# Pablete1234/parquet-floor

Measured on AMD Instinct MI355X. Metric: decoded GB/s + rows/s (node), lineitem-shape Snappy+dict, 1/2/4/8 GPUs, higher is better.
Workload: dtype u8; 1 GPU; lineitem SF1 x1 (6001215 rows x 1, 16 cols, 6 row groups of 1Mi rows), Snappy + dictionary, device-resident; row_groups_per_rank=6, compressed_page_bytes_rank0=217870360

## Files before the change

### parquet-floor_amd/csrc/pf_snappy_par.hip

```cpp
#include <hip/hip_runtime.h>


#include "pf_launch.h"
#include "pf_snappy_par.h"

namespace pf {

#ifdef PF_STAMPS
__device__ unsigned long long pf_stamps[16];
#define STAMP_ADD(i, v) atomicAdd(&pf_stamps[i], (unsigned long long)(v))
__device__ unsigned long long pf_cstamps[32];
#define CSTAMP(i, v) atomicAdd(&pf_cstamps[i], (unsigned long long)(v))
extern "C" int pf_debug_cstamps(unsigned long long* out, int n, int reset) {
    if (hipMemcpyFromSymbol(out, HIP_SYMBOL(pf_cstamps), sizeof(unsigned long long) * (n < 32 ? n : 32)) != hipSuccess) return -1;
    if (reset) {
        unsigned long long z[32] = {};
        if (hipMemcpyToSymbol(HIP_SYMBOL(pf_cstamps), z, sizeof z) != hipSuccess) return -1;
    }
    return 0;
}
#define XT_DECL unsigned long long xt_ = __builtin_amdgcn_s_memtime()
#define XT(i) do { const unsigned long long t_ = __builtin_amdgcn_s_memtime(); if (lane == 0) STAMP_ADD(i, t_ - xt_); xt_ = t_; } while (0)
#else
#define STAMP_ADD(i, v) ((void)0)
// ... 985 lines not shown
        for (uint32_t u = 0; u < XST; u++)
            put16(o, a0 + 16 * u, *reinterpret_cast<const u32x4*>(ring + ((a0 + 16 * u) & XRMASK)));
        F += XSLOT;
        nsl += XST;
    }
    return nsl;
}

__device__ __forceinline__ uint32_t dpp_incl_scan(uint32_t v) {
    v += __builtin_amdgcn_update_dpp(0u, v, 0x111, 0xf, 0xf, false);
    v += __builtin_amdgcn_update_dpp(0u, v, 0x112, 0xf, 0xf, false);
    v += __builtin_amdgcn_update_dpp(0u, v, 0x114, 0xf, 0xf, false);
    v += __builtin_amdgcn_update_dpp(0u, v, 0x118, 0xf, 0xf, false);
    v += __builtin_amdgcn_update_dpp(0u, v, 0x142, 0xa, 0xf, false);
    v += __builtin_amdgcn_update_dpp(0u, v, 0x143, 0xc, 0xf, false);
    return v;
}
__device__ __forceinline__ uint32_t dpp_prev(uint32_t v) {
    return __builtin_amdgcn_update_dpp(0u, v, 0x138, 0xf, 0xf, false);
}

__device__ __forceinline__ void wait_vmem_last_slot() {
    if constexpr (XST == 1) asm volatile("s_waitcnt vmcnt(1)" ::: "memory");
    else asm volatile("s_waitcnt vmcnt(2)" ::: "memory");
}

[[maybe_unused]] constexpr uint32_t X2_STAGE_OFF = XRING;
constexpr uint32_t X2_FBUF_OFF = XRING + ((XSTAGE + 15u) & ~15u);
[[maybe_unused]] constexpr uint32_t X2_LDS = X2_FBUF_OFF + XFAR * FBUF_W * 4;
enum : uint32_t { X2_LDSADDR = 0, X2_COPY = 1 };

#ifdef PF_DIAG
__global__ __launch_bounds__(64) void k_snappy_exec2(const SnappyJob* __restrict__ jobs, const int2* __restrict__ pieces,
                                                     const uint32_t* __restrict__ splits, int* __restrict__ fb, int mode) {
    __shared__ __attribute__((aligned(16))) uint8_t L[X2_LDS];
    __shared__ uint16_t tokpos[XCHUNK / 2];
    __shared__ uint32_t sbits[XBATCH / 32];
    __shared__ uint32_t wpre[XBATCH / 32];
    __shared__ uint16_t jv[256];
    uint8_t* const ring = L;
    uint8_t* const stage = L + X2_STAGE_OFF;
    uint32_t* const fbuf = reinterpret_cast<uint32_t*>(L + X2_FBUF_OFF);
    const int lane = threadIdx.x;
    int j, k;
    if (mode == 0) {
        const int2 pc = pieces[blockIdx.x];
        j = pc.x;
        k = pc.y;
    } else {
        j = blockIdx.x;
        k = 0;
    }
    const int f = fb[j];
    bool whole;
    if (mode == 0) {
        if (f >= FB_REDO || (f == FB_WHOLE && k > 0)) return;
        whole = f == FB_WHOLE;
    } else {
        if (f != FB_REDO) return;
        whole = true;
    }
    const SnappyJob job = jobs[j];
    const uint8_t* in = job.src;
    uint8_t* dst = job.dst;
    const uint64_t n = job.src_len;
    const uint32_t* sp = splits + job.split_base;
    uint64_t pos0 = 0, ulen = 0;
    if (!uvarint(in, n, pos0, ulen) || ulen != job.dst_len) {
        if (lane == 0) atomicMax(&fb[j], FB_SERIAL);
        return;
    }
    if (mode == 0 && (job.dflags & 1u)) {
        if (lane == 0) atomicMax(&fb[j], FB_REDO);
        return;
    }
    uint32_t ip, out_start, out_end = job.dst_len;
    if (whole) {
        ip = uint32_t(pos0);
        out_start = 0;
    } else {
        if (k > 0 && sp[k] == SNAP_INVALID) return;
        ip = k == 0 ? uint32_t(pos0) : sp[k];
        out_start = uint32_t(k) * SNAP_BLOCK;
        for (uint32_t k2 = k + 1; k2 < job.n_pieces; k2++)
            if (sp[k2] != SNAP_INVALID) { out_end = k2 * SNAP_BLOCK; break; }
    }
    const PF_GLOBAL uint16_t* tm16 = (const PF_GLOBAL uint16_t*)(job.tokmap);
    const PF_GLOBAL uint8_t* gin = gptr(in);
    PF_GLOBAL uint8_t* gdst = gptr(dst);
    const OutDst od{gdst, mode == 0 ? gptr(job.ddst) : nullptr, job.dlo, job.dgran};
    uint32_t op = out_start, F = out_start;
    uint32_t nst = 0;
    bool bad = false;
    XT_DECL;
#ifdef PF_STAMPS
    const unsigned long long xt0 = xt_;
    if (lane == 0) STAMP_ADD(13, 1);
#endif
    while (op < out_end && !bad) {
        if (ip >= n) { bad = true; break; }
        const uint32_t I = ip & ~15u;
        __syncthreads();
        const uint32_t woff = snap_stage(stage, in, n, I, XSTAGE, lane);
        const uint32_t p16 = I + 16u * uint32_t(lane);
        uint32_t bits = uint64_t(p16) < n ? uint32_t(tm16[p16 >> 4]) : 0u;
        if (p16 + 16u <= ip) bits = 0;
        else if (p16 < ip) bits &= ~((1u << (ip - p16)) - 1u);
        const uint32_t cnt = __popc(bits);
        const uint32_t ex = dpp_incl_scan(cnt);
        const uint32_t T = __builtin_amdgcn_readlane(ex, 63);
        uint32_t q = ex - cnt;
        while (bits) {
            const uint32_t b = uint32_t(__ffs(bits) - 1);
            bits &= bits - 1;
            tokpos[q++] = uint16_t(16u * uint32_t(lane) + b);
        }
        nst = 0;
        __syncthreads();
        XT(7);
        if (T == 0) { bad = true; break; }
        uint32_t sb = 0;
        while (sb < T && op < out_end) {
            const uint32_t t = sb + uint32_t(lane);
            const bool v = t < T;
            const uint32_t pos = v ? uint32_t(tokpos[t]) : 0u;
            const SnapTok tk = snap_tok(lds_read8(stage, woff + pos));
            const uint32_t ol = v ? tk.ol : 0u;
            const uint32_t start = I + pos;
            const uint32_t endp = tk.tl > uint64_t(0xffffffffu - start) ? 0xffffffffu : start + uint32_t(tk.tl);
            const uint32_t prev = dpp_prev(endp);
            const uint32_t inc = dpp_incl_scan(ol);
            const uint32_t otok = op + inc - ol;
            const bool take = v && otok < out_end;
            const int nt = __popcll(__ballot(take));
            const bool wrong = take && ((lane == 0 ? start != ip : start != prev) || endp > n || op + inc > out_end ||
                                        inc < ol);
            if (__any(wrong)) { bad = true; break; }
            if (nt == 0) break;
            const uint32_t kd = tk.kind;
            const uint32_t off = tk.arg;
            const uint32_t srcv = start + tk.arg;
            const bool lstaged = srcv + ol <= I + XCHUNK + 64;
            const uint32_t a = otok - off;
            const bool farc = take && kd != 0 && a + min(ol, off) <= op && int32_t(a - (op + XBATCH - XRING)) < 0;
            const unsigned long long farm = __ballot(farc);
            const uint32_t frank = uint32_t(__popcll(farm & lane_mask_lt(uint32_t(lane))));
            const unsigned long long cutm = __ballot(take && (ol > 64u || inc > XBATCH || (kd == 0 && !lstaged) ||
                                                              (farc && frank >= XFAR)));
            const uint32_t cut = cutm ? uint32_t(__ffsll(cutm) - 1) : uint32_t(nt);
            uint32_t used, btot;
            XT(1);
            if (lane == 0) STAMP_ADD(0, 1);
            if (cut == 0) {
                const uint32_t L0 = __builtin_amdgcn_readfirstlane(ol);
                const uint32_t s0 = __builtin_amdgcn_readfirstlane(srcv);
                if (__builtin_amdgcn_readfirstlane(kd) != 0) { bad = true; break; }
                uint32_t fl_slots = 0;
                for (uint32_t d0 = 0; d0 < L0; d0 += XLIT) {
                    const uint32_t c = min(L0 - d0, XLIT);
                    const uint32_t b0 = uint32_t(lane) * 16u;
                    if (b0 < c) {
                        uint8_t by[16];
                        #pragma unroll
                        for (int u = 0; u < 16; u++) by[u] = b0 + u < c ? gin[s0 + d0 + b0 + u] : uint8_t(0);
                        #pragma unroll
                        for (int u = 0; u < 16; u++)
                            if (b0 + u < c) ring[(op + d0 + b0 + u) & XRMASK] = by[u];
                    }
                    fl_slots += flush_slots(ring, od, F, op + d0 + c, lane);
                }
                nst = fl_slots;
                used = 1;
                btot = L0;
                XT(11);
            } else {
                used = cut;
                btot = __builtin_amdgcn_readlane(inc, cut - 1);
                const bool inb = take && uint32_t(lane) < cut;
                const bool lit = inb && kd == 0;
                const bool cp = inb && kd != 0;
                if (__any(cp && (off == 0 || off > otok - out_start))) { bad = true; break; }
                const bool far = cp && farc;
                if (od.dd != nullptr && __any(far && a < od.dlo && a + ol > od.dlo)) { bad = true; break; }
                if (__any(far)) {
                    if (nst == XST) wait_vmem_last_slot();
                    else wait_vmem();
                    if (far) {
                        const PF_GLOBAL uint8_t* fb0 = od.dd != nullptr && a >= od.dlo ? od.dd + a : gdst + a;
                        const uintptr_t fa = reinterpret_cast<uintptr_t>(fb0);
                        const PF_GLOBAL uint32_t* fsrc = (const PF_GLOBAL uint32_t*)(fa & ~uintptr_t(3));
                        const uint32_t nwd = (uint32_t(fa & 3u) + ol + 3u) >> 2;
                        uint32_t fw[FBUF_W];
                        #pragma unroll
                        for (int u = 0; u < int(FBUF_W); u++) fw[u] = uint32_t(u) < nwd ? fsrc[u] : 0u;
                        uint32_t* fl = fbuf + frank * FBUF_W;
                        #pragma unroll
                        for (int u = 0; u < int(FBUF_W); u++)
                            if (uint32_t(u) < nwd) fl[u] = fw[u];
                    }
                }
                if (lane == 0 && __any(far)) STAMP_ADD(9, 1);
                XT(3);
                const uint32_t rel = otok - op;
                uint32_t d0 = 0, d1 = 0;
                if (inb) {
                    const bool near = cp && !far;
                    d0 = rel | ((near ? X2_COPY : X2_LDSADDR) << 11) | ((near && off < ol) ? (1u << 12) : 0u) |
                         (min(off, 0xffffu) << 16);
                    const uint32_t fsh = od.dd != nullptr && a >= od.dlo
                                             ? uint32_t((reinterpret_cast<uintptr_t>(od.dd) + a) & 3u) : (a & 3u);
                    d1 = lit ? X2_STAGE_OFF + woff + (srcv - I)
                             : (far ? X2_FBUF_OFF + frank * (FBUF_W * 4) + fsh : a);
                }
                if (lane < int(XBATCH / 32)) sbits[lane] = 0;
                __syncthreads();
                if (inb) atomicOr(&sbits[rel >> 5], 1u << (rel & 31u));
                __syncthreads();
                {
                    const uint32_t c = lane < int(XBATCH / 32) ? __popc(sbits[lane]) : 0u;
                    const uint32_t e2 = dpp_incl_scan(c) - c;
                    if (lane < int(XBATCH / 32)) wpre[lane] = e2;
                }
                __syncthreads();
                XT(4);
                for (uint32_t w0 = 0; w0 < btot; w0 += 256) {
                    if (lane == 0) STAMP_ADD(8, 1);
                    const uint32_t s0 = op + w0;
                    uint32_t W[4], xw[4], ti[4], i0[4], i1[4], addr[4];
                    bool act[4], pend[4];
                    #pragma unroll
                    for (int u = 0; u < 4; u++) {
                        const uint32_t x = w0 + 64u * uint32_t(u) + uint32_t(lane);
                        act[u] = x < btot;
                        xw[u] = act[u] ? x : btot - 1u;
                    }
                    #pragma unroll
                    for (int u = 0; u < 4; u++) {
                        const uint32_t wd = xw[u] >> 5;
                        ti[u] = wpre[wd] + __popc(sbits[wd] & ((2u << (xw[u] & 31u)) - 1u)) - 1u;
                    }
                    #pragma unroll
                    for (int u = 0; u < 4; u++) {
                        i0[u] = uint32_t(__builtin_amdgcn_ds_bpermute(int(ti[u] << 2), int(d0)));
                        i1[u] = uint32_t(__builtin_amdgcn_ds_bpermute(int(ti[u] << 2), int(d1)));
                    }
                    #pragma unroll
                    for (int u = 0; u < 4; u++) {
                        const uint32_t jj = xw[u] - (i0[u] & 0x7ffu);
                        const bool copy = ((i0[u] >> 11) & 1u) == X2_COPY;
                        const uint32_t offv = max(i0[u] >> 16, 1u);
                        const uint32_t r = (i0[u] & (1u << 12)) ? mod_small(jj & 63u, offv) : jj;
                        const uint32_t y = i1[u] + r;
                        pend[u] = act[u] && copy && y >= s0;
                        addr[u] = copy ? (y & XRMASK) : (i1[u] + jj);
                        W[u] = 0x100u | ((y - s0) & 0xffu);
                    }
                    #pragma unroll
                    for (int u = 0; u < 4; u++) {
                        const uint32_t v = uint32_t(L[addr[u]]);
                        W[u] = pend[u] ? W[u] : (act[u] ? v : 0u);
                    }
                    while (__any(((W[0] | W[1] | W[2] | W[3]) & 0x100u) != 0u)) {
                        if (lane == 0) STAMP_ADD(5, 1);
                        #pragma unroll
                        for (int u = 0; u < 4; u++) jv[64u * uint32_t(u) + uint32_t(lane)] = uint16_t(W[u]);
                        uint32_t G[4];
                        #pragma unroll
                        for (int u = 0; u < 4; u++) G[u] = jv[W[u] & 0xffu];
                        #pragma unroll
                        for (int u = 0; u < 4; u++) W[u] = (W[u] & 0x100u) ? G[u] : W[u];
                    }
                    #pragma unroll
                    for (int u = 0; u < 4; u++)
                        if (act[u]) ring[(s0 + 64u * uint32_t(u) + uint32_t(lane)) & XRMASK] = uint8_t(W[u]);
                }
                XT(2);
                const uint32_t sl = flush_slots(ring, od, F, op + btot, lane);
                if (sl) nst = sl;
                XT(6);
            }
            op += btot;
            ip = __builtin_amdgcn_readlane(endp, int(used) - 1);
            sb += used;
        }
    }
    if (bad) {
        if (lane == 0) atomicMax(&fb[j], whole ? FB_SERIAL : FB_REDO);
        return;
    }
#ifdef PF_STAMPS
    if (lane == 0) STAMP_ADD(12, __builtin_amdgcn_s_memtime() - xt0);
#endif
    for (uint32_t a = F + uint32_t(lane) * 16u; a + 16u <= op; a += 1024u)
        put16(od, a, *reinterpret_cast<const u32x4*>(ring + (a & XRMASK)));
    for (uint32_t a = F + ((op - F) & ~15u) + uint32_t(lane); a < op; a += 64) put1(od, a, ring[a & XRMASK]);
}
#endif

#ifndef PF_X5_BATCH
#define PF_X5_BATCH 764
#endif
constexpr uint32_t X5_BATCH = PF_X5_BATCH;
constexpr uint32_t X5_STG = (XSTAGE + 15u) & ~15u;
constexpr uint32_t X5_FSLOT = 80u;
constexpr uint32_t X5_FSL = XFAR * X5_FSLOT;
constexpr uint32_t X5_STAGE0 = XRING;
constexpr uint32_t X5_LDS = XRING + 2u * X5_STG;
constexpr uint32_t X5_W = 768u / 32u;
constexpr uint32_t X5_LINE = 128u;
constexpr uint32_t X5_FREAD = 5u * 16u;
#ifndef PF_X5_TPL
#define PF_X5_TPL 2
#endif
constexpr int X5_TPL = PF_X5_TPL;
constexpr uint32_t X5_DS = 64u * X5_TPL + 1u;
static_assert(X5_BATCH + 3u <= 768u, "a batch and its alignment bytes are at most three 256-byte windows");
static_assert((X5_FSLOT & 15u) == 0u, "far slots are 16-byte aligned");
static_assert(5u * XFAR <= 128u, "a batch's far-copy chunks are loaded by two LDS-DMA wave instructions");
enum : uint32_t { R5_NORMAL = 0, R5_LONG = 1, R5_NOP = 2, R5_END = 3, R5_BAD = 4 };
constexpr uint32_t X5_CP = 0x80000000u;
static_assert(XRING <= 4096u, "ring-copy offsets must stay below 4096: tests/test_exec_arith.py checks (j * m) >> 16 up to there");

__device__ __forceinline__ void x5_barrier() { asm volatile("s_waitcnt lgkmcnt(0)\n\ts_barrier" ::: "memory"); }
__device__ __forceinline__ void x5_order() { asm volatile("" ::: "memory"); }

__device__ __forceinline__ uint32_t x5_pick(uint32_t w, uint32_t g) {
    uint32_t m, r;
    asm("v_pk_ashrrev_i16 %0, 15, %1 op_sel_hi:[0,1]" : "=v"(m) : "v"(w));
    asm("v_bfi_b32 %0, %1, %2, %3" : "=v"(r) : "v"(m), "v"(g), "v"(w));
    return r;
}

struct X5Lds {
    __attribute__((aligned(16))) uint8_t L[X5_LDS];
    uint16_t tokpos[XCHUNK / 2];
    uint32_t D[2][2 * X5_DS];
    uint32_t SB[2][X5_W], WP[2][X5_W];
    uint32_t REC[2][4];
    __attribute__((aligned(8))) uint16_t jv[256];
#if defined(PF_X5_PAD) && PF_X5_PAD > 0
    uint8_t pad[PF_X5_PAD];
#endif
};

__device__ __forceinline__ u32x4 x5_load16(const PF_GLOBAL uint8_t* gin, uint32_t src) {
    const uintptr_t a = reinterpret_cast<uintptr_t>(gin) + src;
    const PF_GLOBAL u32x4* p = (const PF_GLOBAL u32x4*)(a & ~uintptr_t(15));
    const uint32_t sh = uint32_t(a & 15u);
    const u32x4 A = p[0];
    u32x4 B = A;
    if (sh) B = p[1];
    const uint32_t w[8] = {A.x, A.y, A.z, A.w, B.x, B.y, B.z, B.w};
    const uint32_t k = sh >> 2, s = sh & 3u;
    u32x4 r;
    #pragma unroll
    for (int i = 0; i < 4; i++) {
        const uint32_t lo = k == 0 ? w[i] : (k == 1 ? w[i + 1] : (k == 2 ? w[i + 2] : w[i + 3]));
        const uint32_t hi = k == 0 ? w[i + 1] : (k == 1 ? w[i + 2] : (k == 2 ? w[i + 3] : w[i + 4]));
        r[i] = __builtin_amdgcn_alignbyte(hi, lo, s);
    }
    return r;
}

__device__ __forceinline__ void x5_dma16(uint64_t g, uint32_t lds) {
    asm volatile("s_mov_b32 m0, %1\n\ts_nop 0\n\tglobal_load_lds_dwordx4 %0, off" : : "v"(g), "s"(lds) : "memory");
}

static_assert(XSTAGE == 64u * 16u + 5u * 16u, "a staged chunk is 64 + 5 lane loads");
__device__ __forceinline__ void x5_chunk_load(const PF_GLOBAL uint8_t* gin, const PF_GLOBAL uint16_t* tm16, uint64_t n, uint32_t I,
                                              int lane, u32x4& va, u32x4& vb, uint32_t& bits) {
    const uintptr_t a = reinterpret_cast<uintptr_t>(gin + I);
    const uint32_t woff = uint32_t(a & 15u);
    const PF_GLOBAL u32x4* src = (const PF_GLOBAL u32x4*)(a - woff);
    const int64_t first = int64_t(I) - int64_t(woff);
    va = u32x4{0u, 0u, 0u, 0u};
    vb = u32x4{0u, 0u, 0u, 0u};
    bits = 0u;
    if (first + 16 * int64_t(lane) < int64_t(n)) va = src[lane];
    if (lane < 5 && first + 16 * int64_t(64 + lane) < int64_t(n)) vb = src[64 + lane];
    const uint32_t p16 = I + 16u * uint32_t(lane);
    if (uint64_t(p16) < n) bits = uint32_t(tm16[p16 >> 4]);
}

__device__ __forceinline__ void exec5_piece(X5Lds& S, uint8_t* FS, const SnappyJob* __restrict__ jobs, const int2* __restrict__ pieces,
                                            const uint32_t* __restrict__ splits, int* __restrict__ fb, int mode, int item) {
    uint8_t* const L = S.L;
    uint16_t* const tokpos = S.tokpos;
    auto& D = S.D;
    auto& SB = S.SB;
    auto& WP = S.WP;
    auto& REC = S.REC;
    uint8_t* const jvb = reinterpret_cast<uint8_t*>(S.jv);
    uint8_t* const ring = L;
    const uint32_t Lb = uint32_t(reinterpret_cast<uintptr_t>(L));
    const uint32_t FSB = uint32_t(reinterpret_cast<uintptr_t>(FS)) - Lb;
    const int wv = __builtin_amdgcn_readfirstlane(int(threadIdx.x) >> 6);
    const int lane = int(threadIdx.x) & 63;
    int j, k;
    if (mode == 0) {
        const int2 pc = pieces[item];
        j = pc.x;
        k = pc.y;
    } else {
        j = item;
        k = 0;
    }
    const int f = fb[j];
    bool whole;
    if (mode == 0) {
        if (f >= FB_REDO || (f == FB_WHOLE && k > 0)) return;
        whole = f == FB_WHOLE;
    } else {
        if (f != FB_REDO) return;
        whole = true;
    }
    const SnappyJob job = jobs[j];
    const uint8_t* in = job.src;
    const uint64_t n = job.src_len;
    const uint32_t* sp = splits + job.split_base;
    uint64_t pos0 = 0, ulen = 0;
    if (!uvarint(in, n, pos0, ulen) || ulen != job.dst_len) {
        if (threadIdx.x == 0) atomicMax(&fb[j], FB_SERIAL);
        return;
    }
    if (mode == 0 && (job.dflags & 1u)) {
        if (threadIdx.x == 0) atomicMax(&fb[j], FB_REDO);
        return;
    }
    uint32_t ip, out_start, out_end = job.dst_len;
    if (whole) {
        ip = uint32_t(pos0);
        out_start = 0;
    } else {
        if (k > 0 && sp[k] == SNAP_INVALID) return;
        ip = k == 0 ? uint32_t(pos0) : sp[k];
        out_start = uint32_t(k) * SNAP_BLOCK;
        for (uint32_t k2 = k + 1; k2 < job.n_pieces; k2++)
            if (sp[k2] != SNAP_INVALID) { out_end = k2 * SNAP_BLOCK; break; }
    }
    const PF_GLOBAL uint16_t* tm16 = (const PF_GLOBAL uint16_t*)(job.tokmap);
    const PF_GLOBAL uint8_t* gin = gptr(in);
    PF_GLOBAL uint8_t* gdst = gptr(job.dst);
    const OutDst od{gdst, mode == 0 ? gptr(job.ddst) : nullptr, job.dlo, job.dgran};
    if (threadIdx.x < 2) {
        D[threadIdx.x][0] = 0u;
        D[threadIdx.x][X5_DS] = 0u;
    }
    uint32_t op = out_start, sb = 0, T = 0, I = 0, woff = 0, cb = 1;
    uint32_t ops_m1 = out_start, k_m1 = R5_NOP, k_m2 = R5_NOP, nops = 0;
    uint32_t pfI = ~0u, pfbits = 0;
    u32x4 pfa = {0u, 0u, 0u, 0u}, pfb = {0u, 0u, 0u, 0u};
    uint32_t F = out_start, cop = out_start;
    uint32_t last = R5_END;
#ifdef PF_STAMPS
    unsigned long long x5t = __builtin_amdgcn_s_memtime();
#define X5T(i) do { const unsigned long long t_ = __builtin_amdgcn_s_memtime(); if (lane == 0) STAMP_ADD(i, t_ - x5t); x5t = t_; } while (0)
    if (threadIdx.x == 0) STAMP_ADD(13, 1);
#else
#define X5T(i) ((void)0)
#endif
    for (uint32_t it = 0;; it++) {
        const uint32_t b = it & 1u;
        if (wv == 0) {
            if (lane == 0) STAMP_ADD(12, 1);
            uint32_t kind = R5_BAD, b_op = op, b_tot = 0, b_s0 = 0;
            const uint32_t sf = out_start + ((ops_m1 - out_start) & ~(XSLOT - 1u));
            const uint32_t LF = k_m2 == R5_NORMAL ? (sf >= out_start + XSLOT ? sf - XSLOT : out_start) : sf;
            bool ok = true;
            if (op >= out_end) {
                kind = R5_END;
                ok = false;
            } else if (sb >= T) {
                if (ip >= n) {
                    ok = false;
                } else {
                    I = ip & ~15u;
                    cb ^= 1u;
                    u32x4 va, vb;
                    uint32_t bits;
                    if (I == pfI) {
                        va = pfa;
                        vb = pfb;
                        bits = pfbits;
                    } else {
                        x5_chunk_load(gin, tm16, n, I, lane, va, vb, bits);
                    }
                    u32x4* stq = reinterpret_cast<u32x4*>(L + X5_STAGE0 + cb * X5_STG);
                    stq[lane] = va;
                    if (lane < 5) stq[64 + lane] = vb;
                    woff = uint32_t(reinterpret_cast<uintptr_t>(gin + I) & 15u);
                    pfI = I + XCHUNK;
                    if (uint64_t(pfI) < n) x5_chunk_load(gin, tm16, n, pfI, lane, pfa, pfb, pfbits);
                    else pfI = ~0u;
                    const uint32_t p16 = I + 16u * uint32_t(lane);
                    if (p16 + 16u <= ip) bits = 0;
                    else if (p16 < ip) bits &= ~((1u << (ip - p16)) - 1u);
                    const uint32_t cnt = __popc(bits);
                    const uint32_t ex = dpp_incl_scan(cnt);
                    T = __builtin_amdgcn_readlane(ex, 63);
                    uint32_t q = ex - cnt;
                    while (bits) {
                        const uint32_t bb = uint32_t(__ffs(bits) - 1);
                        bits &= bits - 1;
                        tokpos[q++] = uint16_t(16u * uint32_t(lane) + bb);
                    }
                    sb = 0;
                    x5_order();
                    if (T == 0) ok = false;
                }
            }
            X5T(0);
            if (ok) {
                const uint32_t stg_off = __builtin_amdgcn_readfirstlane(cb) ? X5_STAGE0 + X5_STG : X5_STAGE0;
                const uint8_t* stg = L + stg_off;
                uint32_t pos[X5_TPL], ol[X5_TPL], start[X5_TPL], endp[X5_TPL], inc[X5_TPL], otok[X5_TPL];
                bool v[X5_TPL], take[X5_TPL];
                SnapTok32 tk[X5_TPL];
                #pragma unroll
                for (int h = 0; h < X5_TPL; h++) {
                    const uint32_t t = sb + 64u * uint32_t(h) + uint32_t(lane);
                    v[h] = t < T;
                    pos[h] = uint32_t(tokpos[min(t, XCHUNK / 2u - 1u)]);
                    if (!v[h]) pos[h] = 0u;
                }
                uint32_t tlo[X5_TPL], thi[X5_TPL];
                #pragma unroll
                for (int h = 0; h < X5_TPL; h++) lds_read8_2(stg, woff + pos[h], tlo[h], thi[h]);
                #pragma unroll
                for (int h = 0; h < X5_TPL; h++) tk[h] = snap_tok32(tlo[h], thi[h]);
                int nt = 0;
                bool wrong = false;
                uint32_t prevlast = ip, incbase = 0;
                #pragma unroll
                for (int h = 0; h < X5_TPL; h++) {
                    ol[h] = v[h] ? tk[h].ol : 0u;
                    start[h] = I + pos[h];
                    endp[h] = __builtin_elementwise_add_sat(start[h], tk[h].tl);
                    const uint32_t pdpp = dpp_prev(endp[h]);
                    const uint32_t prev = lane == 0 ? prevlast : pdpp;
                    inc[h] = incbase + dpp_incl_scan(ol[h]);
                    otok[h] = op + inc[h] - ol[h];
                    take[h] = v[h] && otok[h] < out_end;
                    nt += __popcll(__ballot(take[h]));
                    wrong = wrong || (take[h] && (start[h] != prev || endp[h] > n || op + inc[h] > out_end || inc[h] < ol[h] ||
                                                  inc[h] < incbase));
                    prevlast = __builtin_amdgcn_readlane(endp[h], 63);
                    incbase = __builtin_amdgcn_readlane(inc[h], 63);
                }
                if (__any(wrong) || nt == 0) {
                    ok = false;
                } else {
                    uint32_t kd[X5_TPL], off[X5_TPL], srcv[X5_TPL], a[X5_TPL], frank[X5_TPL];
                    bool farc[X5_TPL], fnr[X5_TPL], lstaged[X5_TPL];
                    unsigned long long farm[X5_TPL], cutm[X5_TPL];
                    uint32_t fbase = 0;
                    #pragma unroll
                    for (int h = 0; h < X5_TPL; h++) {
                        kd[h] = tk[h].kind;
                        off[h] = tk[h].arg;
                        srcv[h] = start[h] + tk[h].arg;
                        lstaged[h] = srcv[h] + ol[h] <= I + XCHUNK + 64;
                        a[h] = otok[h] - off[h];
                        farc[h] = take[h] && kd[h] != 0 && a[h] + min(ol[h], off[h]) <= op &&
                                  int32_t(a[h] - (op + X5_BATCH - XRING)) < 0;
                        fnr[h] = farc[h] && a[h] + X5_FREAD + X5_LINE > LF;
                        farm[h] = __ballot(farc[h]);
                        frank[h] = fbase + uint32_t(__popcll(farm[h] & lane_mask_lt(uint32_t(lane))));
                        fbase += uint32_t(__popcll(farm[h]));
                        cutm[h] = __ballot(take[h] && (ol[h] > 64u || inc[h] > X5_BATCH || (kd[h] == 0 && !lstaged[h]) ||
                                                       (farc[h] && frank[h] >= XFAR) || fnr[h]));
                    }
                    uint32_t cut = uint32_t(nt);
                    #pragma unroll
                    for (int h = X5_TPL - 1; h >= 0; h--)
                        if (cutm[h]) cut = 64u * uint32_t(h) + uint32_t(__ffsll(cutm[h]) - 1);
                    uint32_t used = 0;
                    if (cut == 0) {
                        if (__builtin_amdgcn_readfirstlane(kd[0]) == 0) {
                            kind = R5_LONG;
                            b_tot = __builtin_amdgcn_readfirstlane(ol[0]);
                            b_s0 = __builtin_amdgcn_readfirstlane(srcv[0]);
                            used = 1;
                            nops = 0;
                        } else if (__builtin_amdgcn_readfirstlane(uint32_t(fnr[0])) && nops < 3) {
                            kind = R5_NOP;
                            nops++;
                        } else {
                            ok = false;
                        }
                    } else {
                        used = cut;
                        const uint32_t ch = (cut - 1u) >> 6;
                        uint32_t btot = 0;
                        #pragma unroll
                        for (int h = 0; h < X5_TPL; h++)
                            if (ch == uint32_t(h)) btot = __builtin_amdgcn_readlane(inc[h], (cut - 1u) & 63u);
                        bool inb[X5_TPL], lit[X5_TPL], cp[X5_TPL], far[X5_TPL];
                        bool bad = false;
                        #pragma unroll
                        for (int h = 0; h < X5_TPL; h++) {
                            inb[h] = take[h] && 64u * uint32_t(h) + uint32_t(lane) < cut;
                            lit[h] = inb[h] && kd[h] == 0;
                            cp[h] = inb[h] && kd[h] != 0;
                            far[h] = cp[h] && farc[h];
                            bad = bad || (cp[h] && (off[h] == 0 || off[h] > otok[h] - out_start));
                            bad = bad || (od.dd != nullptr && far[h] && a[h] < od.dlo && a[h] + ol[h] > od.dlo);
                        }
                        if (__any(bad)) ok = false;
                        X5T(1);
                        if (ok) {
                            uint32_t fsh[X5_TPL];
                            uint32_t nfar = 0;
                            uint64_t* fa = reinterpret_cast<uint64_t*>(FS + b * X5_FSL);
                            #pragma unroll
                            for (int h = 0; h < X5_TPL; h++) {
                                const PF_GLOBAL uint8_t* fb0 = od.dd != nullptr && a[h] >= od.dlo ? od.dd + a[h] : gdst + a[h];
                                fsh[h] = uint32_t(reinterpret_cast<uintptr_t>(fb0) & 15u);
                                if (far[h]) fa[frank[h]] = reinterpret_cast<uintptr_t>(fb0) & ~uintptr_t(15);
                                nfar += uint32_t(__popcll(farm[h] & lane_mask_lt(cut > 64u * uint32_t(h) ? cut - 64u * uint32_t(h) : 0u)));
                            }
                            if (nfar) {
                                x5_order();
                                const uint32_t l0 = uint32_t(lane), f0 = (l0 * 205u) >> 10;
                                const uint64_t s0a = fa[f0] + 16u * (l0 - 5u * f0);
                                uint64_t s1a = 0;
                                if (nfar > 12u) {
                                    const uint32_t l1 = l0 + 64u, f1 = (l1 * 205u) >> 10;
                                    s1a = fa[min(f1, XFAR - 1u)] + 16u * (l1 - 5u * f1);
                                }
                                uint8_t* slots = FS + b * X5_FSL;
                                const uint32_t sl0 = __builtin_amdgcn_readfirstlane(uint32_t(reinterpret_cast<uintptr_t>(slots)));
                                if (l0 < 5u * nfar) x5_dma16(s0a, sl0);
                                if (nfar > 12u && l0 + 64u < 5u * nfar) x5_dma16(s1a, sl0 + 1024u);
                            }
                            X5T(2);
                            if (lane < int(X5_W)) SB[b][lane] = 0;
                            #pragma unroll
                            for (int h = 0; h < X5_TPL; h++) {
                                const uint32_t relS = otok[h] - (op & ~3u);
                                uint32_t d0 = 0, d1 = 0;
                                if (inb[h]) {
                                    const bool near = cp[h] && !far[h];
                                    d0 = relS | (near ? (X5_CP | (off[h] << 16)) : 0u);
                                    d1 = near ? uint32_t(65536.0f * __builtin_amdgcn_rcpf(float(off[h]))) + 1u
                                              : (lit[h] ? stg_off + woff + (srcv[h] - I) - relS
                                                        : FSB + b * X5_FSL + frank[h] * X5_FSLOT + fsh[h] - relS);
                                }
                                D[b][1 + 64 * h + lane] = d0;
                                D[b][1 + X5_DS + 64 * h + lane] = d1;
                                x5_order();
                                if (inb[h]) atomicOr(&SB[b][relS >> 5], 1u << (relS & 31u));
                            }
                            x5_order();
                            const uint32_t c = lane < int(X5_W) ? __popc(SB[b][lane]) : 0u;
                            const uint32_t e2 = dpp_incl_scan(c) - c;
                            if (lane < int(X5_W)) WP[b][lane] = e2;
                            kind = R5_NORMAL;
                            b_tot = btot;
                            nops = 0;
                        }
                    }
                    if (ok && used) {
                        op += b_tot;
                        const uint32_t uh = (used - 1u) >> 6;
                        #pragma unroll
                        for (int h = 0; h < X5_TPL; h++)
                            if (uh == uint32_t(h)) ip = __builtin_amdgcn_readlane(endp[h], (used - 1u) & 63u);
                        sb += used;
                    }
                }
            }
            if (!ok && kind != R5_END) kind = R5_BAD;
            if (lane == 0) {
                REC[b][0] = kind;
                REC[b][1] = b_op;
                REC[b][2] = b_tot;
                REC[b][3] = b_s0;
            }
            asm volatile("s_waitcnt vmcnt(0)" ::: "memory");
            X5T(3);
            k_m2 = k_m1;
            k_m1 = kind;
            ops_m1 = b_op;
        } else if (it > 0) {
            const uint32_t pb = b ^ 1u;
            const uint32_t kind = __builtin_amdgcn_readfirstlane(REC[pb][0]);
            const uint32_t s0 = __builtin_amdgcn_readfirstlane(REC[pb][1]);
            const uint32_t btot = __builtin_amdgcn_readfirstlane(REC[pb][2]);
            if (kind == R5_NORMAL) {
                const uint32_t al = s0 & 3u;
                const uint32_t Sb = s0 - al;
                const uint32_t btS = btot + al;
                const uint32_t* sbw = SB[pb];
                const uint32_t* wpw = WP[pb];
                const uint32_t* Dp = D[pb];
                for (uint32_t w0 = 0; w0 < btS; w0 += 256) {
                    const uint32_t x0 = w0 + 4u * uint32_t(lane);
                    const uint32_t ws = w0 == 0 ? al : w0;
                    const uint32_t wd = x0 >> 5, sh = x0 & 31u;
                    const uint32_t sbv = sbw[wd];
                    const uint32_t t0 = wpw[wd] + __popc(sbv & ((2u << sh) - 1u));
                    const uint32_t nb = sbv >> sh;
                    uint32_t tk[4];
                    tk[0] = t0;
                    tk[1] = t0 + ((nb >> 1) & 1u);
                    tk[2] = tk[1] + ((nb >> 2) & 1u);
                    tk[3] = tk[2] + ((nb >> 3) & 1u);
                    uint32_t d0[4], d1[4];
                    #pragma unroll
                    for (int u = 0; u < 4; u++) {
                        d0[u] = Dp[tk[u]];
                        d1[u] = Dp[tk[u] + X5_DS];
                    }
                    uint32_t addr[4], pw[4];
                    bool pend[4];
                    #pragma unroll
                    for (int u = 0; u < 4; u++) {
                        const uint32_t x = x0 + uint32_t(u);
                        const uint32_t jj = x - (d0[u] & 0xffffu);
                        const bool cp = int32_t(d0[u]) < 0;
                        const uint32_t q = __umul24(jj, d1[u]) >> 16;
                        const uint32_t of = (d0[u] >> 16) & 0x7fffu;
                        uint32_t t;
                        asm("v_mad_u32_u24 %0, %1, %2, %1" : "=v"(t) : "v"(of), "v"(q));
                        const uint32_t y = x - t;
                        pend[u] = cp && int32_t(y) >= int32_t(ws);
                        addr[u] = cp ? ((Sb + y) & XRMASK) : (d1[u] + x);
                        pw[u] = 0x8000u | (y << 1);
                    }
                    uint32_t vv[4];
                    #pragma unroll
                    for (int u = 0; u < 4; u++) vv[u] = uint32_t(*reinterpret_cast<const __attribute__((address_space(3))) uint8_t*>(size_t(Lb + addr[u])));
                    asm volatile("" : "+v"(vv[0]), "+v"(vv[1]), "+v"(vv[2]), "+v"(vv[3]));
                    uint32_t Wa = (pend[0] ? pw[0] : (vv[0] << 1)) | ((pend[1] ? pw[1] : (vv[1] << 1)) << 16);
                    uint32_t Wb = (pend[2] ? pw[2] : (vv[2] << 1)) | ((pend[3] ? pw[3] : (vv[3] << 1)) << 16);
                    while (__any(((Wa | Wb) & 0x80008000u) != 0u)) {
                        *reinterpret_cast<uint2*>(jvb + 8u * uint32_t(lane)) = make_uint2(Wa, Wb);
                        const uint32_t g0 = *reinterpret_cast<const uint16_t*>(jvb + (Wa & 0x1feu));
                        const uint32_t g1 = *reinterpret_cast<const uint16_t*>(jvb + ((Wa >> 16) & 0x1feu));
                        const uint32_t g2 = *reinterpret_cast<const uint16_t*>(jvb + (Wb & 0x1feu));
                        const uint32_t g3 = *reinterpret_cast<const uint16_t*>(jvb + ((Wb >> 16) & 0x1feu));
                        const uint32_t ga = __builtin_amdgcn_perm(g1, g0, 0x05040100u), gb = __builtin_amdgcn_perm(g3, g2, 0x05040100u);
                        Wa = x5_pick(Wa, ga);
                        Wb = x5_pick(Wb, gb);
                    }
                    const uint32_t o4 = __builtin_amdgcn_perm(Wb >> 1, Wa >> 1, 0x06040200u);
                    if (x0 < btS) {
                        const uint32_t ra = (Sb + x0) & XRMASK;
                        if (x0 >= al) {
                            *reinterpret_cast<uint32_t*>(ring + ra) = o4;
                        } else {
                            #pragma unroll
                            for (uint32_t u = 1; u < 4; u++)
                                if (u >= al) ring[ra + u] = uint8_t(o4 >> (8u * u));
                        }
                    }
                }
                X5T(6);
                flush_slots(ring, od, F, s0 + btot, lane);
                cop = s0 + btot;
                X5T(7);
                asm volatile("s_waitcnt vmcnt(1)" ::: "memory");
                X5T(8);
            } else if (kind == R5_LONG) {
                const uint32_t sl = __builtin_amdgcn_readfirstlane(REC[pb][3]);
                const uint32_t e = s0 + btot;
                for (uint32_t base = s0 & ~15u; base < e; base += XLIT) {
                    const uint32_t p = base + 16u * uint32_t(lane);
                    if (p < e) {
                        if (p >= s0 && p + 16u <= e) {
                            *reinterpret_cast<u32x4*>(ring + (p & XRMASK)) = x5_load16(gin, sl + (p - s0));
                        } else {
                            for (uint32_t q = max(p, s0); q < min(p + 16u, e); q++) ring[q & XRMASK] = gin[sl + (q - s0)];
                        }
                    }
                    flush_slots(ring, od, F, min(base + XLIT, e), lane);
                }
                cop = e;
                wait_vmem();
            } else {
                wait_vmem();
            }
        }
        X5T(9);
        x5_barrier();
        if (wv == 0) X5T(4); else X5T(10);
        last = __builtin_amdgcn_readfirstlane(REC[b][0]);
        if (last >= R5_END) break;
    }
    if (last == R5_BAD) {
        if (threadIdx.x == 0) atomicMax(&fb[j], whole ? FB_SERIAL : FB_REDO);
        return;
    }
    if (wv == 1) {
        for (uint32_t a = F + uint32_t(lane) * 16u; a + 16u <= cop; a += 1024u)
            put16(od, a, *reinterpret_cast<const u32x4*>(ring + (a & XRMASK)));
        for (uint32_t a = F + ((cop - F) & ~15u) + uint32_t(lane); a < cop; a += 64) put1(od, a, ring[a & XRMASK]);
    }
#undef X5T
}

__global__ __launch_bounds__(128) void k_snappy_exec5(const SnappyJob* __restrict__ jobs, const int2* __restrict__ pieces,
                                                      const uint32_t* __restrict__ splits, int* __restrict__ fb, int mode) {
    __shared__ X5Lds S;
    __shared__ __attribute__((aligned(16))) uint8_t FS[2 * X5_FSL];
    exec5_piece(S, FS, jobs, pieces, splits, fb, mode, int(blockIdx.x));
}

#ifdef PF_STAMPS
extern "C" int pf_debug_stamps(unsigned long long* out, int n, int reset) {
    if (hipMemcpyFromSymbol(out, HIP_SYMBOL(pf_stamps), sizeof(unsigned long long) * (n < 16 ? n : 16)) != hipSuccess) return -1;
    if (reset) {
        unsigned long long z[16] = {};
        if (hipMemcpyToSymbol(HIP_SYMBOL(pf_stamps), z, sizeof z) != hipSuccess) return -1;
    }
    return 0;
}
#endif

void launch_snappy_parse(const SnappyJob* d_jobs, int n_jobs, const int2* d_wins, int n_wins, SnapWin* d_win,
                         SnapEnt* d_ent, uint32_t* d_lane_out, uint32_t* d_splits, int* d_fb, int max_nwin, hipStream_t s) {
    if (n_jobs <= 0) return;
    hipLaunchKernelGGL(k_snappy_index, dim3(n_wins), dim3(64), 0, s, d_jobs, d_wins, d_win, d_ent, d_lane_out, d_fb);
    const uint32_t cap = uint32_t(std::min(FIX_MAXW, (std::max(max_nwin, 1) + 15) & ~15));
    hipLaunchKernelGGL(k_snappy_chain, dim3(n_jobs), dim3(64), 5 * 4 * cap, s, d_jobs, d_win, (const SnapEnt*)d_ent,
                       d_lane_out, d_fb, cap);
#ifndef PF_REPAIR_GRID
#define PF_REPAIR_GRID (1 << 24)
#endif
    hipLaunchKernelGGL(k_snappy_repair, dim3(std::min(n_wins, PF_REPAIR_GRID)), dim3(64), 0, s, d_jobs, d_wins, n_wins,
                       (const SnapWin*)d_win, d_lane_out, d_fb);
    hipLaunchKernelGGL(k_snappy_splits, dim3(n_jobs), dim3(SP_NT), 0, s, d_jobs, (const SnapWin*)d_win,
                       (const uint32_t*)d_lane_out, d_splits, d_fb);
}

void launch_snappy_exec(const SnappyJob* d_jobs, int n_jobs, const int2* d_pieces, int n_pieces, uint32_t* d_splits,
                        int* d_fb, DevChunkResult* d_res, int exec, hipStream_t s) {
    if (n_jobs <= 0) return;
#ifdef PF_DIAG
    if (exec == 2) {
        hipLaunchKernelGGL(k_snappy_exec2, dim3(n_pieces), dim3(64), 0, s, d_jobs, d_pieces, (const uint32_t*)d_splits, d_fb, 0);
        hipLaunchKernelGGL(k_snappy_exec2, dim3(n_jobs), dim3(64), 0, s, d_jobs, d_pieces, (const uint32_t*)d_splits, d_fb, 1);
    } else
#else
    (void)exec;
#endif
    {
        hipLaunchKernelGGL(k_snappy_exec5, dim3(n_pieces), dim3(128), 0, s, d_jobs, d_pieces, (const uint32_t*)d_splits, d_fb, 0);
        hipLaunchKernelGGL(k_snappy_exec5, dim3(n_jobs), dim3(128), 0, s, d_jobs, d_pieces, (const uint32_t*)d_splits, d_fb, 1);
    }
    launch_snappy_serial(d_jobs, n_jobs, d_fb, d_res, s);
}

void launch_snappy(const SnappyJob* d_jobs, int n_jobs, const int2* d_wins, int n_wins, SnapWin* d_win,
                   SnapEnt* d_ent, uint32_t* d_lane_out, const int2* d_pieces, int n_pieces, uint32_t* d_splits,
                   int* d_fb, DevChunkResult* d_res, int max_nwin, int exec, hipStream_t s) {
    launch_snappy_parse(d_jobs, n_jobs, d_wins, n_wins, d_win, d_ent, d_lane_out, d_splits, d_fb, max_nwin, s);
    launch_snappy_exec(d_jobs, n_jobs, d_pieces, n_pieces, d_splits, d_fb, d_res, exec, s);
}

}
```

Baseline: 393.9 decoded GB/s.

## Size far-copy LDS staging per copy length instead of fixed five-chunk slots

Far copies previously each got a fixed 80-byte slot (five 16-byte chunks), capped at XFAR copies per batch. Now each far copy loads only the chunks it needs, based on its alignment shift and length. A prefix scan packs these chunks into a shared pool of up to 64 (configurable) chunks, so more far copies fit per batch and fewer useless bytes are DMA'd into LDS. The cost is an extra scan, a per-chunk address table write, and more batch cuts when the chunk budget is exceeded.

```diff
diff --git a/parquet-floor_amd/csrc/pf_snappy_par.hip b/parquet-floor_amd/csrc/pf_snappy_par.hip
--- a/parquet-floor_amd/csrc/pf_snappy_par.hip
+++ b/parquet-floor_amd/csrc/pf_snappy_par.hip
@@ -1311,21 +1311,24 @@
 #endif
 constexpr uint32_t X5_BATCH = PF_X5_BATCH;
 constexpr uint32_t X5_STG = (XSTAGE + 15u) & ~15u;
-constexpr uint32_t X5_FSLOT = 80u;
-constexpr uint32_t X5_FSL = XFAR * X5_FSLOT;
+#ifndef PF_X5_FCH
+#define PF_X5_FCH 64
+#endif
+constexpr uint32_t X5_FCH = PF_X5_FCH;
+constexpr uint32_t X5_FSL = X5_FCH * 16u;
 constexpr uint32_t X5_STAGE0 = XRING;
 constexpr uint32_t X5_LDS = XRING + 2u * X5_STG;
 constexpr uint32_t X5_W = 768u / 32u;
 constexpr uint32_t X5_LINE = 128u;
-constexpr uint32_t X5_FREAD = 5u * 16u;
 #ifndef PF_X5_TPL
 #define PF_X5_TPL 2
 #endif
 constexpr int X5_TPL = PF_X5_TPL;
 constexpr uint32_t X5_DS = 64u * X5_TPL + 1u;
 static_assert(X5_BATCH + 3u <= 768u, "a batch and its alignment bytes are at most three 256-byte windows");
-static_assert((X5_FSLOT & 15u) == 0u, "far slots are 16-byte aligned");
-static_assert(5u * XFAR <= 128u, "a batch's far-copy chunks are loaded by two LDS-DMA wave instructions");
+static_assert(X5_FCH <= 128u, "a batch's far-copy chunks are loaded by at most two LDS-DMA wave instructions");
+static_assert(X5_FCH >= 32u && (X5_FCH > 64u ? 128u : 64u) * 8u <= X5_FSL && (X5_FCH + 4u) * 8u <= X5_FSL,
+              "the chunk address table (an entry per loading lane, and four past the last chunk) lies inside one batch's chunk bytes");
 enum : uint32_t { R5_NORMAL = 0, R5_LONG = 1, R5_NOP = 2, R5_END = 3, R5_BAD = 4 };
 constexpr uint32_t X5_CP = 0x80000000u;
 static_assert(XRING <= 4096u, "ring-copy offsets must stay below 4096: tests/test_exec_arith.py checks (j * m) >> 16 up to there");
@@ -1559,10 +1562,10 @@
                 if (__any(wrong) || nt == 0) {
                     ok = false;
                 } else {
-                    uint32_t kd[X5_TPL], off[X5_TPL], srcv[X5_TPL], a[X5_TPL], frank[X5_TPL];
-                    bool farc[X5_TPL], fnr[X5_TPL], lstaged[X5_TPL];
-                    unsigned long long farm[X5_TPL], cutm[X5_TPL];
-                    uint32_t fbase = 0;
+                    uint32_t kd[X5_TPL], off[X5_TPL], srcv[X5_TPL], a[X5_TPL], fsh[X5_TPL], nch[X5_TPL], fce[X5_TPL];
+                    bool farc[X5_TPL], fnr[X5_TPL], lstaged[X5_TPL], fdd[X5_TPL];
+                    unsigned long long cutm[X5_TPL], farm = 0;
+                    unsigned long long wide2 = 0, wide4 = 0;
                     #pragma unroll
                     for (int h = 0; h < X5_TPL; h++) {
                         kd[h] = tk[h].kind;
@@ -1572,13 +1575,44 @@
                         a[h] = otok[h] - off[h];
                         farc[h] = take[h] && kd[h] != 0 && a[h] + min(ol[h], off[h]) <= op &&
                                   int32_t(a[h] - (op + X5_BATCH - XRING)) < 0;
-                        fnr[h] = farc[h] && a[h] + X5_FREAD + X5_LINE > LF;
-                        farm[h] = __ballot(farc[h]);
-                        frank[h] = fbase + uint32_t(__popcll(farm[h] & lane_mask_lt(uint32_t(lane))));
-                        fbase += uint32_t(__popcll(farm[h]));
+                        fnr[h] = farc[h] && a[h] + ol[h] + (X5_LINE - 1u) > LF;
+                        farm |= __ballot(farc[h]);
+                        fsh[h] = 0u;
+                        nch[h] = 0u;
+                        fce[h] = 0u;
+                        fdd[h] = false;
+                    }
+                    if (farm) {
+                        const uint32_t dst_lo = uint32_t(reinterpret_cast<uintptr_t>(gdst)) & 15u;
+                        const uint32_t dd_lo = uint32_t(reinterpret_cast<uintptr_t>(od.dd)) & 15u;
+                        uint32_t anyn = 0;
+                        #pragma unroll
+                        for (int h = 0; h < X5_TPL; h++) {
+                            fdd[h] = od.dd != nullptr && a[h] >= od.dlo;
+                            fsh[h] = ((fdd[h] ? dd_lo : dst_lo) + a[h]) & 15u;
+                            nch[h] = farc[h] ? (fsh[h] + ol[h] + 15u) >> 4 : 0u;
+                            anyn |= nch[h];
+                        }
+                        wide2 = __ballot(anyn > 1u);
+                        wide4 = __ballot(anyn > 3u);
+                        uint32_t cbase = 0;
+                        #pragma unroll
+                        for (int h = 0; h < X5_TPL; h += 2) {
+                            const int h1 = h + 1 < X5_TPL ? h + 1 : h;
+                            const uint32_t sc = dpp_incl_scan(nch[h] | (h1 != h ? nch[h1] << 16 : 0u));
+                            const uint32_t tot = __builtin_amdgcn_readlane(sc, 63);
+                            fce[h] = cbase + (sc & 0xffffu);
+                            cbase += tot & 0xffffu;
+                            if (h1 != h) {
+                                fce[h1] = cbase + (sc >> 16);
+                                cbase += tot >> 16;
+                            }
+                        }
+                    }
+                    #pragma unroll
+                    for (int h = 0; h < X5_TPL; h++)
                         cutm[h] = __ballot(take[h] && (ol[h] > 64u || inc[h] > X5_BATCH || (kd[h] == 0 && !lstaged[h]) ||
-                                                       (farc[h] && frank[h] >= XFAR) || fnr[h]));
-                    }
+                                                       (farc[h] && fce[h] > X5_FCH) || fnr[h]));
                     uint32_t cut = uint32_t(nt);
                     #pragma unroll
                     for (int h = X5_TPL - 1; h >= 0; h--)
@@ -1600,10 +1634,13 @@
                     } else {
                         used = cut;
                         const uint32_t ch = (cut - 1u) >> 6;
-                        uint32_t btot = 0;
+                        uint32_t btot = 0, ntot = 0;
                         #pragma unroll
                         for (int h = 0; h < X5_TPL; h++)
-                            if (ch == uint32_t(h)) btot = __builtin_amdgcn_readlane(inc[h], (cut - 1u) & 63u);
+                            if (ch == uint32_t(h)) {
+                                btot = __builtin_amdgcn_readlane(inc[h], (cut - 1u) & 63u);
+                                ntot = __builtin_amdgcn_readlane(fce[h], (cut - 1u) & 63u);
+                            }
                         bool inb[X5_TPL], lit[X5_TPL], cp[X5_TPL], far[X5_TPL];
                         bool bad = false;
                         #pragma unroll
@@ -1618,29 +1655,33 @@
                         if (__any(bad)) ok = false;
                         X5T(1);
                         if (ok) {
-                            uint32_t fsh[X5_TPL];
-                            uint32_t nfar = 0;
-                            uint64_t* fa = reinterpret_cast<uint64_t*>(FS + b * X5_FSL);
-                            #pragma unroll
-                            for (int h = 0; h < X5_TPL; h++) {
-                                const PF_GLOBAL uint8_t* fb0 = od.dd != nullptr && a[h] >= od.dlo ? od.dd + a[h] : gdst + a[h];
-                                fsh[h] = uint32_t(reinterpret_cast<uintptr_t>(fb0) & 15u);
-                                if (far[h]) fa[frank[h]] = reinterpret_cast<uintptr_t>(fb0) & ~uintptr_t(15);
-                                nfar += uint32_t(__popcll(farm[h] & lane_mask_lt(cut > 64u * uint32_t(h) ? cut - 64u * uint32_t(h) : 0u)));
-                            }
-                            if (nfar) {
+                            if (ntot) {
+                                uint64_t* ca = reinterpret_cast<uint64_t*>(FS + b * X5_FSL);
+                                uint64_t fb0v[X5_TPL];
+                                #pragma unroll
+                                for (int h = 0; h < X5_TPL; h++) {
+                                    const uint64_t fb0 = reinterpret_cast<uintptr_t>((fdd[h] ? od.dd : gdst) + a[h]) & ~uintptr_t(15);
+                                    fb0v[h] = fb0;
+                                }
+                                #pragma unroll
+                                for (int i = 4; i >= 0; i--) {
+                                    if ((i >= 3 && !wide4) || (i >= 1 && !wide2)) continue;
+                                    #pragma unroll
+                                    for (int h = 0; h < X5_TPL; h++)
+                                        if (far[h]) ca[fce[h] - nch[h] + uint32_t(i)] = fb0v[h] + 16u * uint32_t(i);
+                                }
                                 x5_order();
-                                const uint32_t l0 = uint32_t(lane), f0 = (l0 * 205u) >> 10;
-                                const uint64_t s0a = fa[f0] + 16u * (l0 - 5u * f0);
+                                const uint32_t l0 = uint32_t(lane);
+                                uint64_t s0a = ca[l0];
                                 uint64_t s1a = 0;
-                                if (nfar > 12u) {
-                                    const uint32_t l1 = l0 + 64u, f1 = (l1 * 205u) >> 10;
-                                    s1a = fa[min(f1, XFAR - 1u)] + 16u * (l1 - 5u * f1);
-                                }
-                                uint8_t* slots = FS + b * X5_FSL;
-                                const uint32_t sl0 = __builtin_amdgcn_readfirstlane(uint32_t(reinterpret_cast<uintptr_t>(slots)));
-                                if (l0 < 5u * nfar) x5_dma16(s0a, sl0);
-                                if (nfar > 12u && l0 + 64u < 5u * nfar) x5_dma16(s1a, sl0 + 1024u);
+                                if constexpr (X5_FCH > 64u)
+                                    if (ntot > 64u) s1a = ca[64u + l0];
+                                asm volatile("" : "+v"(s0a), "+v"(s1a) :: "memory");
+                                uint8_t* chunks = FS + b * X5_FSL;
+                                const uint32_t sl0 = __builtin_amdgcn_readfirstlane(uint32_t(reinterpret_cast<uintptr_t>(chunks)));
+                                if (l0 < ntot) x5_dma16(s0a, sl0);
+                                if constexpr (X5_FCH > 64u)
+                                    if (ntot > 64u && l0 + 64u < ntot) x5_dma16(s1a, sl0 + 1024u);
                             }
                             X5T(2);
                             if (lane < int(X5_W)) SB[b][lane] = 0;
@@ -1653,7 +1694,7 @@
                                     d0 = relS | (near ? (X5_CP | (off[h] << 16)) : 0u);
                                     d1 = near ? uint32_t(65536.0f * __builtin_amdgcn_rcpf(float(off[h]))) + 1u
                                               : (lit[h] ? stg_off + woff + (srcv[h] - I) - relS
-                                                        : FSB + b * X5_FSL + frank[h] * X5_FSLOT + fsh[h] - relS);
+                                                        : FSB + b * X5_FSL + 16u * (fce[h] - nch[h]) + fsh[h] - relS);
                                 }
                                 D[b][1 + 64 * h + lane] = d0;
                                 D[b][1 + X5_DS + 64 * h + lane] = d1;
```

Result: faster. 407.6 decoded GB/s, median of 6 (+3.5%).
